# karpathy/minbpe

Measured on AMD Instinct MI355X. Metric: BPE merges/sec, higher is better.
Workload: dtype int32; 1 GPU; regex1g: RegexTokenizer.train, 1 GB synth seed 2, vocab 32000; mode=default, parallelism=single

## Files before the change

minbpe_amd/csrc/kernels/k_chain.hip:

```cpp
#include <hip/hip_runtime.h>
#include <stdint.h>

#include "../bpe_device.h"

namespace bpe {
namespace BPE_G {

constexpr uint32_t CH_EX_CAP = 2048;

__device__ __forceinline__ int chain_match(const uint32_t *pa, const uint32_t *pb, uint32_t K, uint32_t w0, uint32_t w1) {
    const uint32_t x = w0 & IDMASK, y = w1 & NWMASK;
    int hit = -1;
    for (uint32_t p = 0; p < K; p++)
        if (x == pa[p] && y == pb[p]) hit = (int)p;
    return (w0 == INVALID_WORD) ? -1 : hit;
}

constexpr uint32_t CH_DCAP = 1024;
constexpr uint32_t CH_SD = 2 * CH_DCAP + 2;
__device__ __forceinline__ void chain_slot_load(const AbArgs &A, const uint32_t t, uint4 (&rv)[MJ], uint4 &hv) {
    const int lane = lane_id();
    const uint32_t *src = A.b0 + (size_t)t * TILE2;
#pragma unroll
    for (int j = 0; j < MJ; j++) rv[j] = *reinterpret_cast<const uint4 *>(src + j * 256 + lane * 4);
    hv = (lane & 1) ? make_uint4(INVALID_WORD, INVALID_WORD, 0u, 0u) : make_uint4(INVALID_WORD, INVALID_WORD, INVALID_WORD, 0u);
    const long long hi = 2ll * (long long)t - 2 + lane;
    if (lane < 6 && hi >= 0 && hi < 2ll * (long long)A.T) hv = reinterpret_cast<const uint4 *>(A.hdr_in)[hi];
}
template <bool DENSE, bool THROUGH = false>
__device__ __forceinline__ void merge_chain_wave(uint32_t *__restrict__ out, uint32_t *__restrict__ sd, const uint32_t t, const AbArgs &A,
                                                 const uint32_t *pa, const uint32_t *pb, const uint32_t *pb1,
                                                 const uint32_t K, const uint32_t z0, const uint32_t brep,
                                                 uint4 (&rv)[MJ], const uint4 hv,
                                                 const uint32_t *ph = nullptr, const uint32_t hm = 0,
                                                 const uint32_t tl_in = 0xFFFFFFFFu) {
    const int lane = lane_id();
    const uint32_t Tl = tl_in != 0xFFFFFFFFu ? tl_in : min(A.T, A.st->tlive);
    const uint32_t *src;
    const uint32_t meta = bcast(hv.w, 2);
    const uint32_t len = meta & 0x7FFFFFFFu, buf = meta >> 31;
    auto keep_header = [&]() {
        if (DENSE && (lane == 2 || lane == 3)) reinterpret_cast<uint4 *>(A.hdr_out)[2 * (size_t)t + (lane - 2)] = hv;
    };
    if (len == 0) {
        keep_header();
        return;
    }
    if (buf) {
        src = A.b1 + (size_t)t * TILE2;
#pragma unroll
        for (int j = 0; j < MJ; j++) rv[j] = *reinterpret_cast<const uint4 *>(src + j * 256 + lane * 4);
    }
    const uint32_t first = bcast(hv.x, 2);
    uint32_t halo0 = bcast(hv.x, 4), halo1 = bcast(hv.y, 4), halo2 = bcast(hv.z, 4);
    uint32_t prev2 = bcast(hv.x, 1), prev1 = bcast(hv.y, 1);
    uint32_t tprev = t - 1;
    uint32_t tnext = t + 1;
    {
        const uint32_t nlen = bcast(hv.w, 4) & 0x7FFFFFFFu, plen = bcast(hv.w, 0) & 0x7FFFFFFFu;
        if ((t + 1 < Tl && nlen < 3) || (t > 0 && plen < 2)) {
            uint32_t ctx[7] = {0, 0, 0, 0, 0, 0, 0};
            if (lane == 0) slot_context_walk(A.hdr_in, t, Tl, ctx);
            halo0 = bcast(ctx[0], 0);
            halo1 = bcast(ctx[1], 0);
            halo2 = bcast(ctx[2], 0);
            prev2 = bcast(ctx[3], 0);
            prev1 = bcast(ctx[4], 0);
            tprev = bcast(ctx[5], 0);
            tnext = bcast(ctx[6], 0);
        }
    }
    auto at = [&](int q, uint32_t own) -> uint32_t {
        const int d = q - (int)len;
        return d < 0 ? own : (d == 0 ? halo0 : (d == 1 ? halo1 : (d == 2 ? halo2 : INVALID_WORD)));
    };
    uint32_t x[MJ][4];
#pragma unroll
    for (int j = 0; j < MJ; j++) {
        const int q0 = j * 256 + lane * 4;
        if ((j + 1) * 256 <= (int)len) {
            x[j][0] = rv[j].x;
            x[j][1] = rv[j].y;
            x[j][2] = rv[j].z;
            x[j][3] = rv[j].w;
        } else {
            x[j][0] = at(q0 + 0, rv[j].x);
            x[j][1] = at(q0 + 1, rv[j].y);
            x[j][2] = at(q0 + 2, rv[j].z);
            x[j][3] = at(q0 + 3, rv[j].w);
        }
    }
    uint32_t tail[3];
#pragma unroll
    for (int i = 0; i < 3; i++) tail[i] = at(TILE2 + i, 0u);
    uint32_t rb[MJ], jc[MJ], valid[MJ];
#pragma unroll
    for (int j = 0; j < MJ; j++) {
        rb[j] = 0;
        jc[j] = 0;
    }
    uint32_t s = 0;
    uint32_t ia[MJ];
#pragma unroll
    for (int j = 0; j < MJ; j++) ia[j] = 0;
    uint32_t ip = 0;
    if (hm) {
        auto code = [&](uint32_t w) -> uint32_t {
            const uint32_t id = w & IDMASK;
            const uint32_t e = ph[(__umul24(id, hm) >> 8) & 255u];
            return (e >> 8) == id ? (e & 255u) : 0u;
        };
#pragma unroll
        for (int j = 0; j < MJ; j++) {
#pragma unroll
            for (int k = 0; k < 4; k++) ia[j] |= code(x[j][k]) << (8 * k);
        }
        ip = code(prev1);
    } else {
        for (uint32_t p = 0; p < K; p++) {
            const uint32_t a = pa[p];
#pragma unroll
            for (int j = 0; j < MJ; j++) {
#pragma unroll
                for (int k = 0; k < 4; k++) ia[j] |= ((x[j][k] & IDMASK) == a) ? (p + 1u) << (8 * k) : 0u;
            }
            ip = ((prev1 & IDMASK) == a) ? p + 1u : ip;
        }
    }
#pragma unroll
    for (int j = 0; j < MJ; j++) {
        const uint32_t up = (j < MJ - 1) ? lane_first(x[(j + 1) % MJ][0]) : tail[0];
        const uint32_t nxw = lane_next(x[j][0], up);
#pragma unroll
        for (int k = 0; k < 4; k++) {
            const uint32_t nxt = (k < 3) ? x[j][k + 1] : nxw;
            const uint32_t i = (ia[j] >> (8 * k)) & 255u;
            const uint32_t m = (uint32_t)((nxt & NWMASK) == pb1[i]);
            rb[j] |= m << k;
            jc[j] |= (m ? i : 0u) << (8 * k);
        }
    }
    s = (uint32_t)((prev1 != INVALID_WORD) & ((first & NWMASK) == pb1[ip]));
#pragma unroll
    for (int j = 0; j < MJ; j++) {
        const int nb = (int)len - (j * 256 + lane * 4);
        valid[j] = nb >= 4 ? 0xFu : (nb <= 0 ? 0u : ((1u << nb) - 1u));
    }
    uint32_t anyr = 0;
#pragma unroll
    for (int j = 0; j < MJ; j++) anyr |= rb[j] & valid[j];
    const bool sites = __any(anyr != 0) != 0;
    if (!sites && !s) {
        keep_header();
        return;
    }
    uint32_t mb[MJ], kb[MJ], ex[MJ], cnt[MJ];
#pragma unroll
    for (int j = 0; j < MJ; j++) {
        mb[j] = rb[j] & valid[j];
        const uint32_t upr = (j > 0) ? ((lane_last(rb[(j + MJ - 1) % MJ]) >> 3) & 1u) : s;
        const uint32_t mp = (uint32_t)dpp_mov<0x138>((int)upr, (int)((rb[j] >> 3) & 1u));
        kb[j] = ~((mb[j] << 1) | mp) & valid[j] & 0xFu;
        cnt[j] = (uint32_t)__popc(kb[j]);
    }
    uint32_t total = 0;
    if constexpr (MJ == 4) {
        const uint32_t i01 = wave_iscan_add(cnt[0] | (cnt[1] << 16));
        const uint32_t i23 = wave_iscan_add(cnt[2] | (cnt[3] << 16));
        const uint32_t t01 = lane_last(i01), t23 = lane_last(i23);
        const uint32_t tot0 = t01 & 0xFFFFu, tot1 = t01 >> 16, tot2 = t23 & 0xFFFFu, tot3 = t23 >> 16;
        ex[0] = (i01 & 0xFFFFu) - cnt[0];
        ex[1] = tot0 + (i01 >> 16) - cnt[1];
        ex[2] = tot0 + tot1 + (i23 & 0xFFFFu) - cnt[2];
        ex[3] = tot0 + tot1 + tot2 + (i23 >> 16) - cnt[3];
        total = tot0 + tot1 + tot2 + tot3;
    } else {
#pragma unroll
        for (int j = 0; j < MJ; j++) {
            const uint32_t inc = wave_iscan_add(cnt[j]);
            ex[j] = total + inc - cnt[j];
            total += lane_last(inc);
        }
    }
    uint32_t fstore = 0;
    if (!s) {
        uint32_t fc = 0x7FFFFFFFu;
#pragma unroll
        for (int j = 0; j < MJ; j++) {
            if (mb[j]) {
                const uint32_t k0 = (uint32_t)__ffs((int)mb[j]) - 1u;
                fc = min(fc, ex[j] + (uint32_t)__popc(kb[j] & ((1u << k0) - 1u)));
            }
        }
        fstore = (uint32_t)wave_min_i32((int)fc) & ~3u;
    }
#pragma unroll
    for (int j = 0; j < MJ; j++) {
        uint32_t o = ex[j];
#pragma unroll
        for (int k = 0; k < 4; k++) {
            if ((kb[j] >> k) & 1u) {
                const uint32_t w = x[j][k];
                const uint32_t z = z0 + ((jc[j] >> (8 * k)) & 255u) - 1u;
                out[o++] = ((mb[j] >> k) & 1u) ? (z | (w & (FLAG | WMASK))) : w;
            }
        }
    }
    __builtin_amdgcn_fence(__ATOMIC_RELEASE, "wavefront");
    __builtin_amdgcn_wave_barrier();
    __builtin_amdgcn_fence(__ATOMIC_ACQUIRE, "wavefront");
    {
        uint32_t *dst = (buf ? A.b1 : A.b0) + (size_t)t * TILE2;
        for (uint32_t i = fstore + (uint32_t)lane * 4; i < total; i += 256)
            *reinterpret_cast<uint4 *>(dst + i) = *reinterpret_cast<const uint4 *>(&out[i]);
    }
    if (lane == 0) {
        uint32_t h[8];
        h[0] = total > 0 ? out[0] : INVALID_WORD;
        h[1] = total > 1 ? out[1] : INVALID_WORD;
        h[2] = total > 2 ? out[2] : INVALID_WORD;
        h[3] = total | (buf << 31);
        h[4] = total > 1 ? out[total - 2] : INVALID_WORD;
        h[5] = total > 0 ? out[total - 1] : INVALID_WORD;
        h[6] = h[7] = 0;
        if (DENSE) {
            reinterpret_cast<uint4 *>(A.hdr_out)[2 * (size_t)t] = make_uint4(h[0], h[1], h[2], h[3]);
            reinterpret_cast<uint4 *>(A.hdr_out)[2 * (size_t)t + 1] = make_uint4(h[4], h[5], 0u, 0u);
        } else {
            stage_put<THROUGH>(A.stage + t, t, h);
            atomicOr(&A.smask[t >> 5], 1u << (t & 31));
        }
        if (total < 3 && t + 1 < Tl) A.st->gap = 1;
    }
    if (!sites) return;
    const uint32_t vc = A.vcap & 0xFFFFFFu;
    uint32_t cm2 = 0, ct0 = 0, ct1 = 0;
    if (bcast(mb[0], 0) & 1u) cm2 = (uint32_t)(chain_match(pa, pb, K, prev2, prev1) + 1);
    const uint32_t cm1 = s ? ip : 0u;
    if (bcast(mb[MJ - 1], 63) & 0xCu) {
        ct0 = (uint32_t)(chain_match(pa, pb, K, tail[0], tail[1]) + 1);
        ct1 = (uint32_t)(chain_match(pa, pb, K, tail[1], tail[2]) + 1);
    }
#pragma unroll
    for (int j = 0; j < MJ; j++) {
        if (!__any(mb[j] != 0)) continue;
        uint32_t upm1, dn0;
        if (j > 0) upm1 = lane_last(x[(j + MJ - 1) % MJ][3]);
        else upm1 = prev1;
        if (j < MJ - 1) dn0 = lane_first(x[(j + 1) % MJ][0]);
        else dn0 = tail[0];
        uint32_t W[7];
        W[0] = (uint32_t)dpp_mov<0x138>((int)upm1, (int)x[j][3]);
        W[1] = x[j][0];
        W[2] = x[j][1];
        W[3] = x[j][2];
        W[4] = x[j][3];
        W[5] = lane_next(x[j][0], dn0);
        W[6] = lane_next(x[j][1], (j < MJ - 1) ? lane_first(x[(j + 1) % MJ][1]) : tail[1]);
        const uint32_t lo_fill = (j > 0) ? (lane_last(jc[(j + MJ - 1) % MJ]) >> 16) : (cm2 | (cm1 << 8));
        const uint32_t hi_fill = (j < MJ - 1) ? (lane_first(jc[(j + 1) % MJ]) & 0xFFFFu) : (ct0 | (ct1 << 8));
        const uint32_t lo = (uint32_t)dpp_mov<0x138>((int)lo_fill, (int)(jc[j] >> 16));
        const uint32_t hi = lane_next(jc[j] & 0xFFFFu, hi_fill);
        const unsigned long long win = (unsigned long long)lo | ((unsigned long long)jc[j] << 16) | ((unsigned long long)hi << 48);
        if (mb[j] == 0) continue;
        uint32_t todo = mb[j];
#pragma unroll
        for (int si = 0; si < 2; si++) {
            if (todo == 0) continue;
            const uint32_t k = (uint32_t)__ffs((int)todo) - 1u;
            todo &= todo - 1u;
            const int q = j * 256 + lane * 4 + (int)k;
            const unsigned long long wk = win >> (8u * k);
            const uint32_t p = ((uint32_t)(wk >> 16) & 255u) - 1u;
            const int li = (int)((uint32_t)wk & 255u) - 1, ri = (int)((uint32_t)(wk >> 32) & 255u) - 1;
            const uint32_t Z = z0 + p;
            uint32_t *dl, *dr;
            if (DENSE) {
                dl = sd + p * CH_SD;
                dr = dl + CH_DCAP;
                atomicAdd(&dl[2 * CH_DCAP + 1], 1u);
            } else {
                if (A.removed) atomicAdd(&A.removed[(p * (uint32_t)CH_RMV + (t & (uint32_t)(CH_RMV - 1))) * REMOVED_STRIDE], 1u);
                dl = A.delta + delta_rep_off(p * (uint32_t)CH_RSTRIDE + (t & (brep - 1u)), vc);
                dr = dl + vc;
            }
            const bool k1 = (k & 1u) != 0, k2 = (k & 2u) != 0;
            const uint32_t wa = k2 ? (k1 ? W[4] : W[3]) : (k1 ? W[2] : W[1]);
            const uint32_t wt = word_weight(wa);
            const uint32_t Lw = k2 ? (k1 ? W[3] : W[2]) : (k1 ? W[1] : W[0]);
            if (!(wa & FLAG) && Lw != INVALID_WORD) {
                if (li != (int)p) {
                    const uint32_t Lseq = (li >= 0 && (uint32_t)li < p) ? z0 + (uint32_t)li : (Lw & IDMASK);
                    atomicAdd(&dl[Lseq], wt);
                    if (!DENSE || A.idx) {
                        const uint32_t Lfin = li >= 0 ? z0 + (uint32_t)li : (Lw & IDMASK);
                        index_add(A.idx, A.istride, t, Lfin, Z);
                        if (q == 0) index_add(A.idx, A.istride, tprev, Lfin, Z);
                    }
                }
            }
            const uint32_t R = k2 ? (k1 ? W[6] : W[5]) : (k1 ? W[4] : W[3]);
            if (!(R & FLAG)) {
                if (ri == (int)p) {
                    if (DENSE) atomicAdd(&dl[2 * CH_DCAP], wt);
                    else atomicAdd(&A.st->badj[p], wt);
                } else {
                    atomicAdd(&dr[(ri >= 0 && (uint32_t)ri < p) ? z0 + (uint32_t)ri : (R & IDMASK)], wt);
                }
                if (!DENSE || A.idx) {
                    const uint32_t y = ri >= 0 ? z0 + (uint32_t)ri : (R & IDMASK);
                    index_add(A.idx, A.istride, t, Z, y);
                    if (q + 2 >= (int)len) index_add(A.idx, A.istride, tnext, Z, y);
                }
            }
        }
    }
}

__device__ __forceinline__ void merge_aa_wave(uint32_t *scr, const uint32_t t, const AbArgs &A, const ChainAa &X, const uint32_t a,
                                              const uint32_t newid, const uint32_t Tl) {
    const int lane = lane_id();
    uint32_t *s_hdr = scr, *s_halo = scr + 8;
    uint4 hv6 = (lane & 1) ? make_uint4(INVALID_WORD, INVALID_WORD, 0u, 0u) : make_uint4(INVALID_WORD, INVALID_WORD, INVALID_WORD, 0u);
    {
        const long long hi = 2ll * (long long)t - 2 + lane;
        if (lane < 6 && hi >= 0 && hi < 2ll * (long long)A.T) hv6 = reinterpret_cast<const uint4 *>(A.hdr_in)[hi];
    }
    const uint32_t mi = bcast(hv6.w, 2);
    const int len = (int)(mi & 0x7FFFFFFFu);
    if (len == 0) return;
    const uint32_t cur = mi >> 31;
    const uint32_t *src = (cur ? A.b1 : A.b0) + (size_t)t * TILE2;
    const uint32_t first = bcast(hv6.x, 2);
    uint32_t halo0 = bcast(hv6.x, 4), halo1 = bcast(hv6.y, 4), halo2 = bcast(hv6.z, 4);
    uint32_t prev1 = bcast(hv6.y, 1);
    uint32_t tnext = t + 1;
    {
        const uint32_t nlen = bcast(hv6.w, 4) & 0x7FFFFFFFu, plen = bcast(hv6.w, 0) & 0x7FFFFFFFu;
        if ((t + 1 < Tl && nlen < 3) || (t > 0 && plen < 2)) {
            uint32_t ctx[7] = {0, 0, 0, 0, 0, 0, 0};
            if (lane == 0) slot_context_walk(A.hdr_in, t, Tl, ctx);
            halo0 = bcast(ctx[0], 0);
            halo1 = bcast(ctx[1], 0);
            halo2 = bcast(ctx[2], 0);
            prev1 = bcast(ctx[4], 0);
            tnext = bcast(ctx[6], 0);
        }
    }
    const uint32_t hw1 = bcast(hv6.y, 2), hw2 = bcast(hv6.z, 2), hl0 = bcast(hv6.x, 3), hl1 = bcast(hv6.y, 3);
    if (lane == 0) {
        s_hdr[0] = first;
        s_hdr[1] = hw1;
        s_hdr[2] = hw2;
        s_hdr[3] = mi;
        s_hdr[4] = hl0;
        s_hdr[5] = hl1;
        s_halo[0] = halo0;
        s_halo[1] = halo1;
        s_halo[2] = halo2;
    }
    SlotRaw raw;
    slot_raw_load<true>(raw, src, len);
    __builtin_amdgcn_fence(__ATOMIC_RELEASE, "wavefront");
// ... 34 lines not shown
                }
                ones += 64;
                nextw = (uint32_t)__shfl((int)xq, 63);
            }
            if (!open || ones < lu) {
                sc = (uint32_t)(ones & 1);
            } else {
                uint32_t su = 0;
                bool got = false;
                for (uint32_t spins = 0; spins < LOOKBACK_SPINS; spins++) {
                    const unsigned long long d = desc_load(&X.sdesc[u]);
                    if ((d >> 42) == (tag >> 42) + (1ull << 20)) {
                        su = (uint32_t)(d & 1u);
                        got = true;
                        break;
                    }
                    __builtin_amdgcn_s_sleep(8);
                }
                failed = !got;
                sc = (uint32_t)(((lu - 1) & 1) == 0) ^ su;
            }
        }
        if (lane == 0) {
            desc_store(&X.sdesc[t], tag | (1ull << 62) | sc);
            if (failed) atomicExch(&A.st->status, ST_LOOKBACK);
        }
        s = sc;
    }
    {
        uint32_t anyr = s;
        const int q0 = lane * 4;
        const int nb = len + 1 - q0;
        const uint32_t keep = nb >= 4 ? 0xFu : (nb <= 0 ? 0u : ((1u << nb) - 1u));
        anyr |= tl.rb[0] & keep;
        if (len == TILE2) anyr |= (uint32_t)(((tl.tail[0] & IDMASK) == a) & ((tl.tail[1] & NWMASK) == a));
        if (!__any(anyr != 0)) return;
    }
    tile_lzscan<true>(tl, nullptr);
    uint32_t kept = 0;
    bool changed = false;
    uint32_t *dst = (cur ? A.b0 : A.b1) + (size_t)t * TILE2;
    tile_rewrite<true, true, 1, true>(tl, s, a, a, newid, dst, nullptr, A.delta, A.vcap, len, &kept, &changed, s_hdr, A.idx,
                                      A.istride, t, tnext, t);
    __builtin_amdgcn_fence(__ATOMIC_RELEASE, "wavefront");
    __builtin_amdgcn_wave_barrier();
    __builtin_amdgcn_fence(__ATOMIC_ACQUIRE, "wavefront");
    if (lane == 0 && changed) {
        uint32_t h[8];
        h[0] = kept > 0 ? s_hdr[0] : INVALID_WORD;
        h[1] = kept > 1 ? s_hdr[1] : INVALID_WORD;
        h[2] = kept > 2 ? s_hdr[2] : INVALID_WORD;
        h[3] = kept | ((cur ^ 1u) << 31);
        h[4] = kept > 1 ? s_hdr[4] : INVALID_WORD;
        h[5] = kept > 0 ? s_hdr[5] : INVALID_WORD;
        h[6] = h[7] = 0;
        stage_put<false>(A.stage + t, t, h);
        atomicOr(&A.smask[t >> 5], 1u << (t & 31));
        atomicAdd(&X.removed[(t & 255u) * REMOVED_STRIDE], (uint32_t)len - kept);
        if (kept < 3 && t + 1 < Tl) A.st->gap = 1;
    }
    __builtin_amdgcn_fence(__ATOMIC_RELEASE, "wavefront");
    __builtin_amdgcn_wave_barrier();
}

__device__ __forceinline__ uint32_t chain_hash_find(const uint32_t *pa, uint32_t K, uint32_t *tab) {
    if (K < 5) return 0u;
    const uint32_t lane = (uint32_t)lane_id(), half = lane >> 5, l = lane & 31u;
    const bool in = l < K;
    const uint32_t a = in ? pa[l] : 0u;
    volatile uint32_t *t = tab + half * 256u;
    for (uint32_t m = 129u; m < 256u; m += 4u) {
        const uint32_t h = (__umul24(a, m + 2u * half) >> 8) & 255u;
        if (in) t[h] = l;
        __builtin_amdgcn_fence(__ATOMIC_RELEASE, "wavefront");
        __builtin_amdgcn_wave_barrier();
        __builtin_amdgcn_fence(__ATOMIC_ACQUIRE, "wavefront");
        const bool clash = in && t[h] != l;
        const unsigned long long cb = __ballot(clash);
        if ((uint32_t)cb == 0u) return m;
        if ((uint32_t)(cb >> 32) == 0u) return m + 2u;
    }
    return 0u;
}
__device__ __forceinline__ uint32_t chain_hash_build(uint32_t *s_ph, uint32_t *s_hm, uint32_t *s_hs, const uint32_t *s_pa, uint32_t K,
                                                     bool pre_ok = false, uint32_t pre_hm = 0) {
    if (threadIdx.x < 256) s_ph[threadIdx.x] = 0xFFFFFFFFu;
    uint32_t hm = pre_hm;
    if (!pre_ok) {
        if (threadIdx.x == 0) *s_hm = 0;
        __syncthreads();
        if (wave_id() == 0) {
            const uint32_t f = chain_hash_find(s_pa, K, s_hs);
            if (lane_id() == 0) *s_hm = f;
        }
        __syncthreads();
        hm = *s_hm;
    } else {
        __syncthreads();
    }
    if (hm && threadIdx.x < K) s_ph[(__umul24(s_pa[threadIdx.x], hm) >> 8) & 255u] = (s_pa[threadIdx.x] << 8) | (threadIdx.x + 1u);
    __syncthreads();
    return hm;
}

struct MergeLds {
    alignas(16) uint32_t s_out[LEAN_MT / 64][TILE2];
    uint32_t s_list[LEAN_SUB * 32];
    uint32_t s_tot[2];
    uint32_t s_pa[CH_KMAX], s_pb[CH_KMAX], s_pb1[CH_KMAX + 1];
    uint32_t s_ph[256], s_hm;
    uint32_t s_hs[512];
};
template <bool THROUGH = false>
__device__ __forceinline__ void merge_chain_body(const AbArgs &A, const uint32_t *__restrict__ idx_dirty, uint32_t use_index,
                                                 MergeLds &L, const uint32_t K, const uint32_t z0, const uint32_t brep,
                                                 const uint32_t blk, const uint32_t nblk, unsigned long long *dbg = nullptr,
                                                 const bool have_st = false, const uint32_t tlive_in = 0, const uint32_t gap_in = 0,
                                                 const bool pre_ok = false, const uint32_t pre_hm = 0, const ChainAa *X = nullptr) {
    auto dstamp = [&](int i) {
        if (dbg && threadIdx.x == 0) dbg[i] = wall_clock64();
    };
    DevState *st = A.st;
    auto &s_out = L.s_out;
    auto &s_list = L.s_list;
    auto &s_tot = L.s_tot;
    auto &s_pa = L.s_pa;
    auto &s_pb = L.s_pb;
    auto &s_pb1 = L.s_pb1;
    const uint32_t hm = chain_hash_build(L.s_ph, &L.s_hm, L.s_hs, s_pa, K, pre_ok, pre_hm);
    const uint32_t *s_ph = L.s_ph;
    const uint32_t Tl = min(A.T, have_st ? tlive_in : st->tlive);
    const uint32_t gap = have_st ? gap_in : st->gap;
    constexpr uint32_t NWV = LEAN_MT / 64;
    AbArgs A1 = A;
    A1.newid = z0;
    const uint32_t a0 = s_pa[0], b0 = s_pb[0];
    const bool aa = MJ == 1 && X != nullptr && X->on && K == 1 && a0 == b0;
    auto do_slot = [&](uint32_t t) {
        if constexpr (MJ == 1) {
            if (aa) {
                merge_aa_wave(s_out[wave_id()], t, A, *X, a0, z0, Tl);
                return;
            }
        }
        if (K == 1) {
            merge_ab_wave<true, true, false, THROUGH>(s_out[wave_id()], nullptr, t, A1, a0, b0, Tl);
        } else {
            uint4 rv[MJ], hv;
            chain_slot_load(A, t, rv, hv);
            merge_chain_wave<false, THROUGH>(s_out[wave_id()], nullptr, t, A, s_pa, s_pb, s_pb1, K, z0, brep, rv, hv, s_ph, hm, Tl);
        }
    };
    if (!(use_index & 1u) || gap != 0) {
        const uint32_t nw = nblk * NWV;
        for (uint32_t t = blk * NWV + wave_id(); t < Tl; t += nw) do_slot(t);
        return;
    }
    dstamp(8);
    const uint32_t nwords = (Tl + 31) / 32;
    const uint32_t per = (nwords + nblk - 1) / nblk;
    const uint32_t wlo = blk * per, whi = min(nwords, wlo + per);
    for (uint32_t sub = wlo; sub < whi; sub += LEAN_SUB) {
        uint32_t mk = 0;
        const uint32_t w = sub + threadIdx.x;
        if (threadIdx.x < LEAN_SUB && w < whi) {
            mk = idx_dirty[w];
            for (uint32_t p = 0; p < K; p++) {
                uint32_t h1, h2, h3;
                pair_hash(s_pa[p], s_pb[p], h1, h2, h3);
                mk |= A.idx[(size_t)h1 * A.istride + w] & A.idx[(size_t)h2 * A.istride + w] &
                      A.idx[(size_t)h3 * A.istride + w];
            }
            if (aa) {
                uint32_t nx = 0;
                if (w + 1 < nwords) {
                    uint32_t h1, h2, h3;
                    pair_hash(a0, a0, h1, h2, h3);
                    nx = idx_dirty[w + 1] | (A.idx[(size_t)h1 * A.istride + w + 1] & A.idx[(size_t)h2 * A.istride + w + 1] &
                                             A.idx[(size_t)h3 * A.istride + w + 1]);
                }
                mk |= (mk >> 1) | (nx << 31);
            }
            const uint32_t left = Tl - w * 32;
            if (left < 32) mk &= (1u << left) - 1u;
        }
        const uint32_t c = (uint32_t)__popc(mk);
        const uint32_t inc = wave_iscan_add(c);
        if (threadIdx.x < 128 && lane_id() == 63) s_tot[wave_id()] = inc;
        __syncthreads();
        const uint32_t n = s_tot[0] + s_tot[1];
        if (threadIdx.x < LEAN_SUB) {
            uint32_t o = inc - c + (wave_id() == 1 ? s_tot[0] : 0u);
            while (mk) {
                s_list[o++] = w * 32 + (uint32_t)__ffs((int)mk) - 1u;
                mk &= mk - 1u;
            }
        }
        __syncthreads();
        if (sub == wlo) dstamp(9);
        if (K == 1 || MJ > 1 || !(use_index & 2u)) {
            for (uint32_t i = wave_id(); i < n; i += NWV) do_slot(s_list[i]);
        } else {
            uint32_t i = wave_id();
            uint4 rv[MJ], hv, nrv[MJ], nhv;
            if (i < n) chain_slot_load(A, s_list[i], rv, hv);
            for (; i < n; i += NWV) {
                const bool more = i + NWV < n;
                if (more) chain_slot_load(A, s_list[i + NWV], nrv, nhv);
                merge_chain_wave<false, THROUGH>(s_out[wave_id()], nullptr, s_list[i], A, s_pa, s_pb, s_pb1, K, z0, brep, rv, hv, s_ph, hm, Tl);
                if (more) {
#pragma unroll
                    for (int j = 0; j < MJ; j++) rv[j] = nrv[j];
                    hv = nhv;
                }
            }
        }
        __syncthreads();
    }
}
enum { SW_BB = CH_KMAX, SW_BADJ = 2 * CH_KMAX, SW_BK = 3 * CH_KMAX, SW_BZ0, SW_BREP, SW_STATUS, SW_DEFER, SW_SEL_RAN, SW_TLIVE, SW_GAP, SW_BHM, SW_BHM_KEY, SW_ADJ, SW_N };
constexpr int SW_WORDS = 128;
static_assert(SW_N <= SW_WORDS, "two waves fetch the state words");
__device__ __forceinline__ void step_words_fetch(const DevState *st, uint32_t *s_w) {
    const uint32_t i = threadIdx.x;
    if (i < (uint32_t)SW_N) {
        const uint32_t *base = reinterpret_cast<const uint32_t *>(st);
        uint32_t off;
        if (i < (uint32_t)SW_BB) off = (uint32_t)offsetof(DevState, ba) / 4 + i;
        else if (i < (uint32_t)SW_BADJ) off = (uint32_t)offsetof(DevState, bb) / 4 + (i - (uint32_t)SW_BB);
        else if (i < (uint32_t)SW_BK) off = (uint32_t)offsetof(DevState, badj) / 4 + (i - (uint32_t)SW_BADJ);
        else {
            constexpr uint32_t o[SW_N - SW_BK] = {
                (uint32_t)offsetof(DevState, bk) / 4,      (uint32_t)offsetof(DevState, bz0) / 4,     (uint32_t)offsetof(DevState, brep) / 4,
                (uint32_t)offsetof(DevState, status) / 4,  (uint32_t)offsetof(DevState, defer) / 4,   (uint32_t)offsetof(DevState, sel_ran) / 4,
                (uint32_t)offsetof(DevState, tlive) / 4,   (uint32_t)offsetof(DevState, gap) / 4,     (uint32_t)offsetof(DevState, bhm) / 4,
                (uint32_t)offsetof(DevState, bhm_key) / 4, (uint32_t)offsetof(DevState, adj) / 4};
            off = o[0];
#pragma unroll
            for (int k = 1; k < SW_N - SW_BK; k++) off = (i == (uint32_t)SW_BK + (uint32_t)k) ? o[k] : off;
        }
        s_w[i] = base[off];
    }
    __syncthreads();
}
__global__ void __launch_bounds__(LEAN_MT)
k_merge_chain(AbArgs A, const uint32_t *__restrict__ idx_dirty, uint32_t use_index, uint32_t *__restrict__ dbits, ChainAa X) {
    __shared__ MergeLds L;
    __shared__ uint32_t s_w[SW_WORDS];
    DevState *st = A.st;
    step_words_fetch(st, s_w);
    const uint32_t ran = s_w[SW_SEL_RAN];
    if (blockIdx.x == 0 && ran) {
        for (uint32_t i = threadIdx.x; i < DBITS_WORDS; i += LEAN_MT) dbits[i] = 0;
        __syncthreads();
        if (threadIdx.x == 0) st->sel_ran = 0;
    }
    const uint32_t K = s_w[SW_BK];
    if (s_w[SW_STATUS] || s_w[SW_DEFER] || K == 0) return;
    const uint32_t z0 = s_w[SW_BZ0], brep = s_w[SW_BREP];
    if (threadIdx.x < CH_KMAX) {
        L.s_pa[threadIdx.x] = threadIdx.x < K ? s_w[threadIdx.x] : 0xFFFFFFFFu;
        L.s_pb[threadIdx.x] = threadIdx.x < K ? s_w[SW_BB + threadIdx.x] : 0xFFFFFFFFu;
        L.s_pb1[threadIdx.x + 1] = threadIdx.x < K ? s_w[SW_BB + threadIdx.x] : 0xFFFFFFFFu;
        if (threadIdx.x == 0) L.s_pb1[0] = 0xFFFFFFFFu;
    }
    __syncthreads();
    if (K == 1 && s_w[0] == s_w[SW_BB] && !(MJ == 1 && X.on)) {
        if (blockIdx.x == 0 && threadIdx.x == 0) atomicExch(&st->status, ST_INTERNAL);
        return;
    }
    merge_chain_body(A, idx_dirty, use_index, L, K, z0, brep, blockIdx.x, gridDim.x, nullptr, true, s_w[SW_TLIVE], s_w[SW_GAP],
                     s_w[SW_BHM_KEY] == ((z0 << 8) | K), s_w[SW_BHM], &X);
}

constexpr int CH_KDENSE = 6;
static_assert((LEAN_MT / 64) * TILE2 * 4 + CH_KDENSE * (int)CH_SD * 4 + 256 <= 160 * 1024, "dense chain pass: LDS");
__global__ void __launch_bounds__(LEAN_MT)
k_merge_chain_dense(AbArgs A, uint32_t *__restrict__ dbits) {
    __shared__ __attribute__((aligned(16))) uint32_t s_out[LEAN_MT / 64][TILE2];
    __shared__ uint32_t s_sd[CH_KDENSE * CH_SD];
    __shared__ uint32_t s_pa[CH_KMAX], s_pb[CH_KMAX], s_pb1[CH_KMAX + 1];
    DevState *st = A.st;
    const uint32_t ran = st->sel_ran;
    if (blockIdx.x == 0 && ran) {
        for (uint32_t i = threadIdx.x; i < DBITS_WORDS; i += LEAN_MT) dbits[i] = 0;
        __syncthreads();
        if (threadIdx.x == 0) st->sel_ran = 0;
    }
    const uint32_t K = st->bk;
    if (!(st->status || st->defer) && K == 1) return;
    if (st->status || st->defer || K == 0 || K > (uint32_t)CH_KDENSE) {
        const uint4 *hi = reinterpret_cast<const uint4 *>(A.hdr_in);
        uint4 *ho = reinterpret_cast<uint4 *>(A.hdr_out);
        for (size_t i = (size_t)blockIdx.x * LEAN_MT + threadIdx.x; i < 2 * (size_t)A.T; i += (size_t)gridDim.x * LEAN_MT) ho[i] = hi[i];
        if (K > (uint32_t)CH_KDENSE && blockIdx.x == 0 && threadIdx.x == 0) st->status = ST_INTERNAL;
        return;
    }
    const uint32_t z0 = st->bz0, brep = st->brep;
    if (threadIdx.x < CH_KMAX) {
        s_pa[threadIdx.x] = threadIdx.x < K ? (uint32_t)st->ba[threadIdx.x] : 0xFFFFFFFFu;
        s_pb[threadIdx.x] = threadIdx.x < K ? (uint32_t)st->bb[threadIdx.x] : 0xFFFFFFFFu;
        s_pb1[threadIdx.x + 1] = threadIdx.x < K ? (uint32_t)st->bb[threadIdx.x] : 0xFFFFFFFFu;
        if (threadIdx.x == 0) s_pb1[0] = 0xFFFFFFFFu;
    }
    for (uint32_t i = threadIdx.x; i < K * CH_SD; i += LEAN_MT) s_sd[i] = 0;
    __syncthreads();
    constexpr uint32_t NWV = LEAN_MT / 64;
    const uint32_t nw = gridDim.x * NWV;
    const uint32_t Tl = min(A.T, st->tlive);
    for (uint32_t t = blockIdx.x * NWV + wave_id(); t < A.T; t += nw)
    {
        uint4 rv[MJ], hv;
        chain_slot_load(A, t, rv, hv);
        merge_chain_wave<true>(s_out[wave_id()], s_sd, t, A, s_pa, s_pb, s_pb1, K, z0, (uint32_t)CH_RSTRIDE, rv, hv, nullptr, 0, Tl);
    }
    __syncthreads();
    const uint32_t vc = A.vcap & 0xFFFFFFu;
    const uint32_t lim = min(vc, (uint32_t)CH_DCAP);
    for (uint32_t p = 0; p < K; p++) {
        const uint32_t *sd = s_sd + p * CH_SD;
        uint32_t *g = A.delta + delta_rep_off(p * (uint32_t)CH_RSTRIDE + (blockIdx.x & (brep - 1u)), vc);
        for (uint32_t i = threadIdx.x; i < lim; i += LEAN_MT) {
            const uint32_t l = sd[i], r = sd[CH_DCAP + i];
            if (l) atomicAdd(&g[i], l);
            if (r) atomicAdd(&g[vc + i], r);
        }
        if (threadIdx.x == 0) {
            const uint32_t adj = sd[2 * CH_DCAP], rem = sd[2 * CH_DCAP + 1];
            if (adj) atomicAdd(&st->badj[p], adj);
            if (rem && A.removed) atomicAdd(&A.removed[(p * (uint32_t)CH_RMV + (blockIdx.x & (uint32_t)(CH_RMV - 1))) * REMOVED_STRIDE], rem);
        }
    }
}
__global__ void __launch_bounds__(MT, 5)
k_merge_chain_dense1(AbArgs A) {
    __shared__ __attribute__((aligned(16))) uint32_t s_out[MT / 64][TILE2];
    __shared__ uint32_t s_delta[2 * LDSD_CAP + 2];
    const DevState *st = A.st;
    if (st->status || st->defer || st->bk != 1) return;
    const uint32_t a = (uint32_t)st->ba[0], b = (uint32_t)st->bb[0];
    A.newid = st->bz0;
    ldsd_clear(s_delta);
    const uint32_t nw = gridDim.x * (MT / 64);
    const uint32_t Tl = min(A.T, st->tlive);
    for (uint32_t t = blockIdx.x * (MT / 64) + wave_id(); t < A.T; t += nw)
        merge_ab_wave<false, false, true>(s_out[wave_id()], s_delta, t, A, a, b, Tl);
    ldsd_flush(s_delta, A);
}

template <bool OWNED>
__device__ __forceinline__ void apply_chain_tokens(const uint32_t t, uint32_t *__restrict__ mat, uint32_t stride,
                                                   uint32_t *__restrict__ delta, uint32_t vcap, const uint32_t *__restrict__ rowmax,
                                                   uint32_t *__restrict__ dbits, uint4 *__restrict__ sums,
                                                   const uint32_t *__restrict__ folded, uint32_t fS, const uint32_t *__restrict__ ftail,
                                                   const uint32_t K, const uint32_t z0, const uint32_t ran,
                                                   const uint32_t *pairs, const uint32_t *adjs, const uint32_t brep_in) {
    auto dld = [&](const uint32_t *p) -> uint32_t { return OWNED ? ld_agent(p) : *p; };
    auto pair_a = [&](uint32_t p) -> uint32_t { return pairs[p] >> 16; };
    auto pair_b = [&](uint32_t p) -> uint32_t { return pairs[p] & 0xFFFFu; };
    {
        const uint32_t Zlast = z0 + K - 1u;
        if ((t & ~255u) > Zlast) return;
        const bool live = t <= Zlast;
        const uint32_t nrep = 1u << (vcap >> 24);
        const uint32_t vc = vcap & 0xFFFFFFu;
        uint2 rm = make_uint2(0u, 0u);
        uint32_t prevflag = 0, oldword = 0;
        if (OWNED) {
            oldword = ran ? 0u : dbits[t >> 5];
            prevflag = (oldword >> (t & 31)) & 1u;
            if (live) {
                const unsigned long long v = ld_agent64(reinterpret_cast<const unsigned long long *>(rowmax) + t);
                rm = make_uint2((uint32_t)v, (uint32_t)(v >> 32));
            }
        } else if (live) {
            prevflag = (dbits[t >> 5] >> (t & 31)) & 1u;
            rm = reinterpret_cast<const uint2 *>(rowmax)[t];
        }
        bool flagged = false;
        if (!OWNED && K == 1 && pair_a(0) == pair_b(0)) {
            const uint32_t a = pair_a(0), Z = z0;
            constexpr int RB = 4;
            uint32_t acc[4] = {0, 0, 0, 0};
            const uint32_t old_ta = live ? mat[(size_t)t * stride + a] : 0u;
            for (uint32_t r0 = 0; r0 < nrep; r0 += RB) {
                uint32_t x[RB][4];
#pragma unroll
                for (int k = 0; k < RB; k++)
#pragma unroll
                    for (int v = 0; v < 4; v++)
                        x[k][v] = (live && r0 + k < nrep) ? delta[delta_rep_off(r0 + k, vc) + (size_t)v * vc + t] : 0u;
#pragma unroll
                for (int k = 0; k < RB; k++)
#pragma unroll
                    for (int v = 0; v < 4; v++) {
                        if (x[k][v]) delta[delta_rep_off(r0 + k, vc) + (size_t)v * vc + t] = 0;
                        acc[v] += x[k][v];
// ... 413 lines not shown
```

minbpe_amd/csrc/kernels/k_slots2.hip:

```cpp
#include <hip/hip_runtime.h>
#include <stdint.h>

#include "../bpe_device.h"

namespace bpe {
namespace BPE_G {



__global__ void __launch_bounds__(256)
k_slot2_init(SlotHdr *__restrict__ hdr, uint64_t T, DevState *st, int par, uint32_t which,
             const uint32_t *__restrict__ ids) {
    const uint64_t n = st->n[par];
    if (blockIdx.x == 0 && threadIdx.x == 0) {
        st->gap = 0;
        st->tlive = (uint32_t)min(T, (n + TILE2 - 1) / TILE2);
    }
    const uint64_t stride = (uint64_t)gridDim.x * blockDim.x;
    for (uint64_t t = (uint64_t)blockIdx.x * blockDim.x + threadIdx.x; t < T; t += stride) {
        const uint64_t b0 = t * TILE2;
        const uint32_t len = b0 >= n ? 0u : (uint32_t)min((uint64_t)TILE2, n - b0);
        SlotHdr h;
        h.w0 = len > 0 ? ids[b0] : INVALID_WORD;
        h.w1 = len > 1 ? ids[b0 + 1] : INVALID_WORD;
        h.w2 = len > 2 ? ids[b0 + 2] : INVALID_WORD;
        h.meta = len | (which << 31);
        h.l0 = len > 1 ? ids[b0 + len - 2] : INVALID_WORD;
        h.l1 = len > 0 ? ids[b0 + len - 1] : INVALID_WORD;
        h.pad0 = h.pad1 = 0;
        hdr[t] = h;
    }
}

__device__ __forceinline__ void slot_context_walk(const SlotHdr *__restrict__ hdr, uint32_t t, uint32_t T,
                                                  uint32_t *ctx) {
    uint32_t h0 = INVALID_WORD, h1 = INVALID_WORD, h2 = INVALID_WORD;
    uint32_t tn = 0xFFFFFFFFu;
    int got = 0;
    for (uint32_t u = t + 1; u < T && got < 3; u++) {
        const SlotHdr hh = hdr[u];
        const uint32_t lu = hh.meta & 0x7FFFFFFFu;
        if (lu && tn == 0xFFFFFFFFu) tn = u;
#pragma unroll
        for (uint32_t i = 0; i < 3; i++) {
            if (i < lu && got < 3) {
                const uint32_t w = i == 0 ? hh.w0 : (i == 1 ? hh.w1 : hh.w2);
                if (got == 0) h0 = w;
                else if (got == 1) h1 = w;
                else h2 = w;
                got++;
            }
        }
    }
    uint32_t p1 = INVALID_WORD, p2 = INVALID_WORD, tp = 0xFFFFFFFFu;
    got = 0;
    for (uint32_t u = t; u-- > 0 && got < 2;) {
        const SlotHdr hh = hdr[u];
        const uint32_t lu = hh.meta & 0x7FFFFFFFu;
        if (lu == 0) continue;
        if (got == 0) {
            p1 = hh.l1;
            tp = u;
            got = 1;
            if (lu >= 2) {
                p2 = hh.l0;
                got = 2;
            }
        } else {
            p2 = hh.l1;
            got = 2;
        }
    }
    ctx[0] = h0;
    ctx[1] = h1;
    ctx[2] = h2;
    ctx[3] = p2;
    ctx[4] = p1;
    ctx[5] = tp;
    ctx[6] = tn;
}

__device__ __forceinline__ uint32_t bcast(uint32_t v, int srclane) {
    return (uint32_t)__builtin_amdgcn_readlane((int)v, srclane);
}

template <bool SPARSE, bool INDEXED, bool LDSD, bool THROUGH = false>
__device__ __forceinline__ void merge_ab_wave(uint32_t *__restrict__ out, uint32_t *__restrict__ sd, const uint32_t t,
                                              const AbArgs &A, const uint32_t a, const uint32_t b,
                                              const uint32_t tl_in = 0xFFFFFFFFu) {
    const int lane = lane_id();
    const uint32_t Tl = tl_in != 0xFFFFFFFFu ? tl_in : min(A.T, A.st->tlive);
    const uint32_t *src = A.b0 + (size_t)t * TILE2;
    uint4 rv[MJ];
#pragma unroll
    for (int j = 0; j < MJ; j++) rv[j] = *reinterpret_cast<const uint4 *>(src + j * 256 + lane * 4);
    uint4 hv = (lane & 1) ? make_uint4(INVALID_WORD, INVALID_WORD, 0u, 0u)
                          : make_uint4(INVALID_WORD, INVALID_WORD, INVALID_WORD, 0u);
    {
        const long long hi = 2ll * (long long)t - 2 + lane;
        if (lane < 6 && hi >= 0 && hi < 2ll * (long long)A.T) hv = reinterpret_cast<const uint4 *>(A.hdr_in)[hi];
    }
    const uint32_t meta = bcast(hv.w, 2);
    const uint32_t len = meta & 0x7FFFFFFFu, buf = meta >> 31;
    auto keep_header = [&]() {
        if (!SPARSE && (lane == 2 || lane == 3)) reinterpret_cast<uint4 *>(A.hdr_out)[2 * (size_t)t + (lane - 2)] = hv;
    };
    if (len == 0) {
        keep_header();
        return;
    }
    if (buf) {
        src = A.b1 + (size_t)t * TILE2;
#pragma unroll
        for (int j = 0; j < MJ; j++) rv[j] = *reinterpret_cast<const uint4 *>(src + j * 256 + lane * 4);
    }
    const uint32_t first = bcast(hv.x, 2);
    uint32_t halo0 = bcast(hv.x, 4), halo1 = bcast(hv.y, 4), halo2 = bcast(hv.z, 4);
    uint32_t prev2 = bcast(hv.x, 1), prev1 = bcast(hv.y, 1);
    uint32_t tprev = t - 1;
    uint32_t tnext = t + 1;
    {
        const uint32_t nlen = bcast(hv.w, 4) & 0x7FFFFFFFu, plen = bcast(hv.w, 0) & 0x7FFFFFFFu;
        if ((t + 1 < Tl && nlen < 3) || (t > 0 && plen < 2)) {
            uint32_t ctx[7] = {0, 0, 0, 0, 0, 0, 0};
            if (lane == 0) slot_context_walk(A.hdr_in, t, Tl, ctx);
            halo0 = bcast(ctx[0], 0);
            halo1 = bcast(ctx[1], 0);
            halo2 = bcast(ctx[2], 0);
            prev2 = bcast(ctx[3], 0);
            prev1 = bcast(ctx[4], 0);
            tprev = bcast(ctx[5], 0);
            tnext = bcast(ctx[6], 0);
        }
    }
    auto at = [&](int q, uint32_t own) -> uint32_t {
        const int d = q - (int)len;
        return d < 0 ? own : (d == 0 ? halo0 : (d == 1 ? halo1 : (d == 2 ? halo2 : INVALID_WORD)));
    };
    uint32_t x[MJ][4];
#pragma unroll
    for (int j = 0; j < MJ; j++) {
        const int q0 = j * 256 + lane * 4;
        if ((j + 1) * 256 <= (int)len) {
            x[j][0] = rv[j].x;
            x[j][1] = rv[j].y;
            x[j][2] = rv[j].z;
            x[j][3] = rv[j].w;
        } else {
            x[j][0] = at(q0 + 0, rv[j].x);
            x[j][1] = at(q0 + 1, rv[j].y);
            x[j][2] = at(q0 + 2, rv[j].z);
            x[j][3] = at(q0 + 3, rv[j].w);
        }
    }
    uint32_t tail[3];
#pragma unroll
    for (int i = 0; i < 3; i++) tail[i] = at(TILE2 + i, 0u);
    uint32_t rb[MJ], valid[MJ];
    uint32_t anyr = 0;
#pragma unroll
    for (int j = 0; j < MJ; j++) {
        const uint32_t up = (j < MJ - 1) ? lane_first(x[(j + 1) % MJ][0]) : tail[0];
        const uint32_t nx = lane_next(x[j][0], up);
        uint32_t r = 0;
#pragma unroll
        for (int k = 0; k < 4; k++) {
            const uint32_t nxt = (k < 3) ? x[j][k + 1] : nx;
            r |= (uint32_t)(((x[j][k] & IDMASK) == a) & ((nxt & NWMASK) == b)) << k;
        }
        const int nb = (int)len - (j * 256 + lane * 4);
        valid[j] = nb >= 4 ? 0xFu : (nb <= 0 ? 0u : ((1u << nb) - 1u));
        rb[j] = r;
        anyr |= r & valid[j];
    }
    const uint32_t s = (uint32_t)((prev1 != INVALID_WORD) & ((prev1 & IDMASK) == a) & ((first & NWMASK) == b));
    const bool sites = __any(anyr != 0) != 0;
    if (!sites && !s) {
        keep_header();
        return;
    }
    uint32_t mb[MJ], kb[MJ], ex[MJ], cnt[MJ];
#pragma unroll
    for (int j = 0; j < MJ; j++) {
        mb[j] = rb[j] & valid[j];
        const uint32_t upr = (j > 0) ? ((lane_last(rb[(j + MJ - 1) % MJ]) >> 3) & 1u) : s;
        const uint32_t mp = (uint32_t)dpp_mov<0x138>((int)upr, (int)((rb[j] >> 3) & 1u));
        kb[j] = ~((mb[j] << 1) | mp) & valid[j] & 0xFu;
        cnt[j] = (uint32_t)__popc(kb[j]);
    }
    uint32_t total = 0;
    if constexpr (MJ == 4) {
        const uint32_t i01 = wave_iscan_add(cnt[0] | (cnt[1] << 16));
        const uint32_t i23 = wave_iscan_add(cnt[2] | (cnt[3] << 16));
        const uint32_t t01 = lane_last(i01), t23 = lane_last(i23);
        const uint32_t tot0 = t01 & 0xFFFFu, tot1 = t01 >> 16, tot2 = t23 & 0xFFFFu, tot3 = t23 >> 16;
        ex[0] = (i01 & 0xFFFFu) - cnt[0];
        ex[1] = tot0 + (i01 >> 16) - cnt[1];
        ex[2] = tot0 + tot1 + (i23 & 0xFFFFu) - cnt[2];
        ex[3] = tot0 + tot1 + tot2 + (i23 >> 16) - cnt[3];
        total = tot0 + tot1 + tot2 + tot3;
    } else {
#pragma unroll
        for (int j = 0; j < MJ; j++) {
            const uint32_t inc = wave_iscan_add(cnt[j]);
            ex[j] = total + inc - cnt[j];
            total += lane_last(inc);
        }
    }
    uint32_t fstore = 0;
    if (!s) {
        uint32_t fc = 0x7FFFFFFFu;
#pragma unroll
        for (int j = 0; j < MJ; j++) {
            if (mb[j]) {
                const uint32_t k0 = (uint32_t)__ffs((int)mb[j]) - 1u;
                fc = min(fc, ex[j] + (uint32_t)__popc(kb[j] & ((1u << k0) - 1u)));
            }
        }
        fstore = (uint32_t)wave_min_i32((int)fc) & ~3u;
    }
#pragma unroll
    for (int j = 0; j < MJ; j++) {
        uint32_t o = ex[j];
#pragma unroll
        for (int k = 0; k < 4; k++) {
            if ((kb[j] >> k) & 1u) {
                const uint32_t w = x[j][k];
                out[o++] = ((mb[j] >> k) & 1u) ? (A.newid | (w & (FLAG | WMASK))) : w;
            }
        }
    }
    __builtin_amdgcn_fence(__ATOMIC_RELEASE, "wavefront");
    __builtin_amdgcn_wave_barrier();
    __builtin_amdgcn_fence(__ATOMIC_ACQUIRE, "wavefront");
    {
        uint32_t *dst = (buf ? A.b1 : A.b0) + (size_t)t * TILE2;
        for (uint32_t i = fstore + (uint32_t)lane * 4; i < total; i += 256)
            *reinterpret_cast<uint4 *>(dst + i) = *reinterpret_cast<const uint4 *>(&out[i]);
    }
    if (lane == 0) {
// ... 513 lines not shown
```

Measured before the change: 56740 merges/s.

## Use direct-indexed LDS lookup table and fused pair hash in chain merge

The dense chain merge now builds a direct-mapped LDS table indexed by left token id, holding the right token and pair index. Site detection becomes one lookup per word instead of a hash lookup followed by a second pb1 lookup. The hashed path stores the right token alongside the key in a uint2 entry so the match check is fused into one load. It also packs pair codes with a byte permute, refactors halo placement into helpers, and makes the dense removed-counter atomic conditional on A.removed. In exchange it uses extra LDS for the table, and any left id at or above CH_DCAP falls to a sentinel slot.

Result: no change. 57630 merges/s, median of 6 (+1.6%).

```diff
diff --git a/minbpe_amd/csrc/kernels/k_chain.hip b/minbpe_amd/csrc/kernels/k_chain.hip
--- a/minbpe_amd/csrc/kernels/k_chain.hip
+++ b/minbpe_amd/csrc/kernels/k_chain.hip
@@ -32,8 +32,8 @@
                                                  const uint32_t *pa, const uint32_t *pb, const uint32_t *pb1,
                                                  const uint32_t K, const uint32_t z0, const uint32_t brep,
                                                  uint4 (&rv)[MJ], const uint4 hv,
-                                                 const uint32_t *ph = nullptr, const uint32_t hm = 0,
-                                                 const uint32_t tl_in = 0xFFFFFFFFu) {
+                                                 const uint2 *ph = nullptr, const uint32_t hm = 0,
+                                                 const uint32_t tl_in = 0xFFFFFFFFu, const uint32_t *dt = nullptr) {
     const int lane = lane_id();
     const uint32_t Tl = tl_in != 0xFFFFFFFFu ? tl_in : min(A.T, A.st->tlive);
     const uint32_t *src;
@@ -70,29 +70,18 @@
             tnext = bcast(ctx[6], 0);
         }
     }
-    auto at = [&](int q, uint32_t own) -> uint32_t {
-        const int d = q - (int)len;
-        return d < 0 ? own : (d == 0 ? halo0 : (d == 1 ? halo1 : (d == 2 ? halo2 : INVALID_WORD)));
-    };
     uint32_t x[MJ][4];
 #pragma unroll
     for (int j = 0; j < MJ; j++) {
-        const int q0 = j * 256 + lane * 4;
-        if ((j + 1) * 256 <= (int)len) {
-            x[j][0] = rv[j].x;
-            x[j][1] = rv[j].y;
-            x[j][2] = rv[j].z;
-            x[j][3] = rv[j].w;
-        } else {
-            x[j][0] = at(q0 + 0, rv[j].x);
-            x[j][1] = at(q0 + 1, rv[j].y);
-            x[j][2] = at(q0 + 2, rv[j].z);
-            x[j][3] = at(q0 + 3, rv[j].w);
-        }
+        x[j][0] = rv[j].x;
+        x[j][1] = rv[j].y;
+        x[j][2] = rv[j].z;
+        x[j][3] = rv[j].w;
+        if ((j + 1) * 256 > (int)len) halo_place(x, j, len, halo0, halo1, halo2);
     }
     uint32_t tail[3];
 #pragma unroll
-    for (int i = 0; i < 3; i++) tail[i] = at(TILE2 + i, 0u);
+    for (int i = 0; i < 3; i++) tail[i] = halo_tail(TILE2 + i - (int)len, halo0, halo1, halo2);
     uint32_t rb[MJ], jc[MJ], valid[MJ];
 #pragma unroll
     for (int j = 0; j < MJ; j++) {
@@ -100,23 +89,52 @@
         jc[j] = 0;
     }
     uint32_t s = 0;
-    uint32_t ia[MJ];
-#pragma unroll
-    for (int j = 0; j < MJ; j++) ia[j] = 0;
     uint32_t ip = 0;
-    if (hm) {
-        auto code = [&](uint32_t w) -> uint32_t {
-            const uint32_t id = w & IDMASK;
-            const uint32_t e = ph[(__umul24(id, hm) >> 8) & 255u];
-            return (e >> 8) == id ? (e & 255u) : 0u;
+    if constexpr (DENSE) {
+        auto ent = [&](uint32_t w) -> uint32_t { return dt[min(w & IDMASK, CH_DCAP)]; };
+#pragma unroll
+        for (int j = 0; j < MJ; j++) {
+            const uint32_t up = (j < MJ - 1) ? lane_first(x[(j + 1) % MJ][0]) : tail[0];
+            const uint32_t nxw = lane_next(x[j][0], up);
+#pragma unroll
+            for (int k = 0; k < 4; k++) {
+                const uint32_t nxt = (k < 3) ? x[j][k + 1] : nxw;
+                const uint32_t e = ent(x[j][k]);
+                const bool m = (nxt & NWMASK) == (e >> 8);
+                rb[j] |= (m ? 1u : 0u) << k;
+                jc[j] = code_put(jc[j], m ? e : 0u, k);
+            }
+        }
+        const uint32_t e = ent(prev1);
+        ip = e & 255u;
+        s = (uint32_t)((prev1 != INVALID_WORD) & ((first & NWMASK) == (e >> 8)));
+    } else if (hm) {
+        auto ent = [&](uint32_t w, uint32_t &id) -> uint2 {
+            id = w & IDMASK;
+            return ph[(__umul24(id, hm) >> 8) & 255u];
         };
 #pragma unroll
         for (int j = 0; j < MJ; j++) {
-#pragma unroll
-            for (int k = 0; k < 4; k++) ia[j] |= code(x[j][k]) << (8 * k);
-        }
-        ip = code(prev1);
+            const uint32_t up = (j < MJ - 1) ? lane_first(x[(j + 1) % MJ][0]) : tail[0];
+            const uint32_t nxw = lane_next(x[j][0], up);
+#pragma unroll
+            for (int k = 0; k < 4; k++) {
+                const uint32_t nxt = (k < 3) ? x[j][k + 1] : nxw;
+                uint32_t id;
+                const uint2 e = ent(x[j][k], id);
+                const bool m = ((e.x >> 8) == id) & ((nxt & NWMASK) == e.y);
+                rb[j] |= (m ? 1u : 0u) << k;
+                jc[j] = code_put(jc[j], m ? e.x : 0u, k);
+            }
+        }
+        uint32_t id;
+        const uint2 e = ent(prev1, id);
+        ip = (e.x >> 8) == id ? (e.x & 255u) : 0u;
+        s = (uint32_t)((prev1 != INVALID_WORD) & (ip != 0u) & ((first & NWMASK) == e.y));
     } else {
+        uint32_t ia[MJ];
+#pragma unroll
+        for (int j = 0; j < MJ; j++) ia[j] = 0;
         for (uint32_t p = 0; p < K; p++) {
             const uint32_t a = pa[p];
 #pragma unroll
@@ -126,21 +144,21 @@
             }
             ip = ((prev1 & IDMASK) == a) ? p + 1u : ip;
         }
-    }
-#pragma unroll
-    for (int j = 0; j < MJ; j++) {
-        const uint32_t up = (j < MJ - 1) ? lane_first(x[(j + 1) % MJ][0]) : tail[0];
-        const uint32_t nxw = lane_next(x[j][0], up);
-#pragma unroll
-        for (int k = 0; k < 4; k++) {
-            const uint32_t nxt = (k < 3) ? x[j][k + 1] : nxw;
-            const uint32_t i = (ia[j] >> (8 * k)) & 255u;
-            const uint32_t m = (uint32_t)((nxt & NWMASK) == pb1[i]);
-            rb[j] |= m << k;
-            jc[j] |= (m ? i : 0u) << (8 * k);
-        }
-    }
-    s = (uint32_t)((prev1 != INVALID_WORD) & ((first & NWMASK) == pb1[ip]));
+#pragma unroll
+        for (int j = 0; j < MJ; j++) {
+            const uint32_t up = (j < MJ - 1) ? lane_first(x[(j + 1) % MJ][0]) : tail[0];
+            const uint32_t nxw = lane_next(x[j][0], up);
+#pragma unroll
+            for (int k = 0; k < 4; k++) {
+                const uint32_t nxt = (k < 3) ? x[j][k + 1] : nxw;
+                const uint32_t i = (ia[j] >> (8 * k)) & 255u;
+                const uint32_t m = (uint32_t)((nxt & NWMASK) == pb1[i]);
+                rb[j] |= m << k;
+                jc[j] |= (m ? i : 0u) << (8 * k);
+            }
+        }
+        s = (uint32_t)((prev1 != INVALID_WORD) & ((first & NWMASK) == pb1[ip]));
+    }
 #pragma unroll
     for (int j = 0; j < MJ; j++) {
         const int nb = (int)len - (j * 256 + lane * 4);
@@ -278,7 +296,7 @@
             if (DENSE) {
                 dl = sd + p * CH_SD;
                 dr = dl + CH_DCAP;
-                atomicAdd(&dl[2 * CH_DCAP + 1], 1u);
+                if (A.removed) atomicAdd(&dl[2 * CH_DCAP + 1], 1u);
             } else {
                 if (A.removed) atomicAdd(&A.removed[(p * (uint32_t)CH_RMV + (t & (uint32_t)(CH_RMV - 1))) * REMOVED_STRIDE], 1u);
                 dl = A.delta + delta_rep_off(p * (uint32_t)CH_RSTRIDE + (t & (brep - 1u)), vc);
@@ -479,9 +497,9 @@
     }
     return 0u;
 }
-__device__ __forceinline__ uint32_t chain_hash_build(uint32_t *s_ph, uint32_t *s_hm, uint32_t *s_hs, const uint32_t *s_pa, uint32_t K,
-                                                     bool pre_ok = false, uint32_t pre_hm = 0) {
-    if (threadIdx.x < 256) s_ph[threadIdx.x] = 0xFFFFFFFFu;
+__device__ __forceinline__ uint32_t chain_hash_build(uint2 *s_ph, uint32_t *s_hm, uint32_t *s_hs, const uint32_t *s_pa, const uint32_t *s_pb,
+                                                     uint32_t K, bool pre_ok = false, uint32_t pre_hm = 0) {
+    if (threadIdx.x < 256) s_ph[threadIdx.x] = make_uint2(0xFFFFFFFFu, 0xFFFFFFFFu);
     uint32_t hm = pre_hm;
     if (!pre_ok) {
         if (threadIdx.x == 0) *s_hm = 0;
@@ -495,7 +513,8 @@
     } else {
         __syncthreads();
     }
-    if (hm && threadIdx.x < K) s_ph[(__umul24(s_pa[threadIdx.x], hm) >> 8) & 255u] = (s_pa[threadIdx.x] << 8) | (threadIdx.x + 1u);
+    if (hm && threadIdx.x < K)
+        s_ph[(__umul24(s_pa[threadIdx.x], hm) >> 8) & 255u] = make_uint2((s_pa[threadIdx.x] << 8) | (threadIdx.x + 1u), s_pb[threadIdx.x]);
     __syncthreads();
     return hm;
 }
@@ -505,7 +524,8 @@
     uint32_t s_list[LEAN_SUB * 32];
     uint32_t s_tot[2];
     uint32_t s_pa[CH_KMAX], s_pb[CH_KMAX], s_pb1[CH_KMAX + 1];
-    uint32_t s_ph[256], s_hm;
+    alignas(8) uint2 s_ph[256];
+    uint32_t s_hm;
     uint32_t s_hs[512];
 };
 template <bool THROUGH = false>
@@ -524,8 +544,8 @@
     auto &s_pa = L.s_pa;
     auto &s_pb = L.s_pb;
     auto &s_pb1 = L.s_pb1;
-    const uint32_t hm = chain_hash_build(L.s_ph, &L.s_hm, L.s_hs, s_pa, K, pre_ok, pre_hm);
-    const uint32_t *s_ph = L.s_ph;
+    const uint32_t hm = chain_hash_build(L.s_ph, &L.s_hm, L.s_hs, s_pa, s_pb, K, pre_ok, pre_hm);
+    const uint2 *s_ph = L.s_ph;
     const uint32_t Tl = min(A.T, have_st ? tlive_in : st->tlive);
     const uint32_t gap = have_st ? gap_in : st->gap;
     constexpr uint32_t NWV = LEAN_MT / 64;
@@ -671,11 +691,13 @@
 }
 
 constexpr int CH_KDENSE = 6;
-static_assert((LEAN_MT / 64) * TILE2 * 4 + CH_KDENSE * (int)CH_SD * 4 + 256 <= 160 * 1024, "dense chain pass: LDS");
+static_assert((LEAN_MT / 64) * TILE2 * 4 + CH_KDENSE * (int)CH_SD * 4 + ((int)CH_DCAP + 1) * 4 + 3 * (CH_KMAX + 1) * 4 <= 160 * 1024,
+              "dense chain pass: LDS");
 __global__ void __launch_bounds__(LEAN_MT)
 k_merge_chain_dense(AbArgs A, uint32_t *__restrict__ dbits) {
     __shared__ __attribute__((aligned(16))) uint32_t s_out[LEAN_MT / 64][TILE2];
     __shared__ uint32_t s_sd[CH_KDENSE * CH_SD];
+    __shared__ uint32_t s_dt[CH_DCAP + 1];
     __shared__ uint32_t s_pa[CH_KMAX], s_pb[CH_KMAX], s_pb1[CH_KMAX + 1];
     DevState *st = A.st;
     const uint32_t ran = st->sel_ran;
@@ -701,6 +723,9 @@
         if (threadIdx.x == 0) s_pb1[0] = 0xFFFFFFFFu;
     }
     for (uint32_t i = threadIdx.x; i < K * CH_SD; i += LEAN_MT) s_sd[i] = 0;
+    for (uint32_t i = threadIdx.x; i <= CH_DCAP; i += LEAN_MT) s_dt[i] = 0xFFFFFF00u;
+    __syncthreads();
+    if (threadIdx.x < K && s_pa[threadIdx.x] < CH_DCAP) s_dt[s_pa[threadIdx.x]] = (s_pb[threadIdx.x] << 8) | (threadIdx.x + 1u);
     __syncthreads();
     constexpr uint32_t NWV = LEAN_MT / 64;
     const uint32_t nw = gridDim.x * NWV;
@@ -709,7 +734,7 @@
     {
         uint4 rv[MJ], hv;
         chain_slot_load(A, t, rv, hv);
-        merge_chain_wave<true>(s_out[wave_id()], s_sd, t, A, s_pa, s_pb, s_pb1, K, z0, (uint32_t)CH_RSTRIDE, rv, hv, nullptr, 0, Tl);
+        merge_chain_wave<true>(s_out[wave_id()], s_sd, t, A, s_pa, s_pb, s_pb1, K, z0, (uint32_t)CH_RSTRIDE, rv, hv, nullptr, 0, Tl, s_dt);
     }
     __syncthreads();
     const uint32_t vc = A.vcap & 0xFFFFFFu;
diff --git a/minbpe_amd/csrc/kernels/k_slots2.hip b/minbpe_amd/csrc/kernels/k_slots2.hip
--- a/minbpe_amd/csrc/kernels/k_slots2.hip
+++ b/minbpe_amd/csrc/kernels/k_slots2.hip
@@ -82,6 +82,21 @@
 
 __device__ __forceinline__ uint32_t bcast(uint32_t v, int srclane) {
     return (uint32_t)__builtin_amdgcn_readlane((int)v, srclane);
+}
+__device__ __forceinline__ void halo_place(uint32_t (&x)[MJ][4], const int j, const uint32_t len, const uint32_t h0,
+                                           const uint32_t h1, const uint32_t h2) {
+    const uint32_t lane = (uint32_t)lane_id();
+#pragma unroll
+    for (int k = 0; k < 4; k++) {
+        const int dd = j * 256 + (int)lane * 4 + k - (int)len;
+        x[j][k] = dd < 0 ? x[j][k] : (dd == 0 ? h0 : (dd == 1 ? h1 : (dd == 2 ? h2 : INVALID_WORD)));
+    }
+}
+__device__ __forceinline__ uint32_t halo_tail(const int d, const uint32_t h0, const uint32_t h1, const uint32_t h2) {
+    return d == 0 ? h0 : (d == 1 ? h1 : (d == 2 ? h2 : INVALID_WORD));
+}
+__device__ __forceinline__ uint32_t code_put(const uint32_t jc, const uint32_t v, const int k) {
+    return __builtin_amdgcn_perm(v, jc, 0x03020100u ^ ((4u ^ (uint32_t)k) << (8 * k)));
 }
 
 template <bool SPARSE, bool INDEXED, bool LDSD, bool THROUGH = false>
@@ -133,29 +148,18 @@
             tnext = bcast(ctx[6], 0);
         }
     }
-    auto at = [&](int q, uint32_t own) -> uint32_t {
-        const int d = q - (int)len;
-        return d < 0 ? own : (d == 0 ? halo0 : (d == 1 ? halo1 : (d == 2 ? halo2 : INVALID_WORD)));
-    };
     uint32_t x[MJ][4];
 #pragma unroll
     for (int j = 0; j < MJ; j++) {
-        const int q0 = j * 256 + lane * 4;
-        if ((j + 1) * 256 <= (int)len) {
-            x[j][0] = rv[j].x;
-            x[j][1] = rv[j].y;
-            x[j][2] = rv[j].z;
-            x[j][3] = rv[j].w;
-        } else {
-            x[j][0] = at(q0 + 0, rv[j].x);
-            x[j][1] = at(q0 + 1, rv[j].y);
-            x[j][2] = at(q0 + 2, rv[j].z);
-            x[j][3] = at(q0 + 3, rv[j].w);
-        }
+        x[j][0] = rv[j].x;
+        x[j][1] = rv[j].y;
+        x[j][2] = rv[j].z;
+        x[j][3] = rv[j].w;
+        if ((j + 1) * 256 > (int)len) halo_place(x, j, len, halo0, halo1, halo2);
     }
     uint32_t tail[3];
 #pragma unroll
-    for (int i = 0; i < 3; i++) tail[i] = at(TILE2 + i, 0u);
+    for (int i = 0; i < 3; i++) tail[i] = halo_tail(TILE2 + i - (int)len, halo0, halo1, halo2);
     uint32_t rb[MJ], valid[MJ];
     uint32_t anyr = 0;
 #pragma unroll
```
